# bitsauce/Carla-ppo

Measured on NVIDIA H100. Metric: VAE frames/sec @ batch 4096, higher is better.
Workload: dtype f32

## Files before the change

carla_ppo_b200/csrc/tc_wgrad.cu:

```cuda
#include "tc_common.cuh"
#include "wgrad.cuh"

namespace cpb {

namespace {

using namespace tc;

constexpr int CHUNK_KB = 4;

template <int BN, int PASSES>
struct TcWgCfg {
    static constexpr int B_TILE_BYTES = BN * TBK * 4;
    static constexpr int PARTS = PASSES == 3 ? 2 : 1;
    static constexpr int B_OFF = PARTS * A_TILE_BYTES;
    static constexpr int STAGE_BYTES = PARTS * A_TILE_BYTES + PARTS * B_TILE_BYTES;
    static constexpr int STAGES = (STAGE_BYTES * 4 <= 200 * 1024) ? 4 : 3;
    static constexpr int SMEM_BYTES = STAGES * STAGE_BYTES + 1024;
};

constexpr int kWgLoaderWarps = 8;
constexpr int kWgBWarps = 4;
constexpr int kWgThreads = (kWgLoaderWarps + kWgBWarps) * 32;

template <int BN, int PASSES>
__global__ void __maxnreg__(168)
tc_wgrad_kernel(const __grid_constant__ WgradParams p) {
    static_assert(PASSES == 3 || PASSES == 1, "3xTF32 or a single TF32 pass");
    using Cfg = TcWgCfg<BN, PASSES>;
    constexpr int STAGES = Cfg::STAGES;
    constexpr int B_TILE_BYTES = Cfg::B_TILE_BYTES;
    constexpr int B_OFF = Cfg::B_OFF;
    constexpr int STAGE_BYTES = Cfg::STAGE_BYTES;

    extern __shared__ uint8_t smem_raw[];
    __shared__ uint64_t full_bar[STAGES];
    __shared__ uint64_t empty_bar[STAGES];

    const int tid = threadIdx.x;
    const int warp = __shfl_sync(0xffffffffu, tid >> 5, 0), lane = tid & 31;
    const int i0 = blockIdx.x * TBM;
    const int j0 = blockIdx.y * BN;
    const int HoWo = p.Ho * p.Wo;
    const long long M = (long long)p.batch * HoWo;
    const long long m_begin = (long long)blockIdx.z * p.m_per_split;
    long long m_end = m_begin + p.m_per_split;
    if (m_end > M) m_end = M;
    const int nkb = m_end > m_begin ? 2 * (int)((m_end - m_begin + 2 * TBK - 1) / (2 * TBK)) : 0;

    const uint32_t smem_base = (smem_u32(smem_raw) + 1023u) & ~1023u;
    if (tid == 0) {
#pragma unroll
        for (int s = 0; s < STAGES; ++s) { mbar_init(&full_bar[s], kWgLoaderWarps + kWgBWarps); mbar_init(&empty_bar[s], kWgLoaderWarps); }
        asm volatile("fence.mbarrier_init.release.cluster;" ::: "memory");
    }
    __syncthreads();
    constexpr int BQ = BN / 4;
    const int len = (int)(m_end - m_begin);
    auto store_t = [&](uint32_t tile_hi, uint32_t tile_lo, const float4* x, const uint32_t* so) {
        const float xs[4][4] = {{x[0].x, x[1].x, x[2].x, x[3].x}, {x[0].y, x[1].y, x[2].y, x[3].y},
                                {x[0].z, x[1].z, x[2].z, x[3].z}, {x[0].w, x[1].w, x[2].w, x[3].w}};
#pragma unroll
        for (int c = 0; c < 4; ++c) {
            if constexpr (PASSES == 3) {
                float4 hi, lo;
                split_tf32(xs[c][0], hi.x, lo.x); split_tf32(xs[c][1], hi.y, lo.y);
                split_tf32(xs[c][2], hi.z, lo.z); split_tf32(xs[c][3], hi.w, lo.w);
                asm volatile("st.shared.v4.f32 [%0], {%1,%2,%3,%4};" ::"r"(tile_hi + so[c]), "f"(hi.x), "f"(hi.y), "f"(hi.z), "f"(hi.w) : "memory");
                asm volatile("st.shared.v4.f32 [%0], {%1,%2,%3,%4};" ::"r"(tile_lo + so[c]), "f"(lo.x), "f"(lo.y), "f"(lo.z), "f"(lo.w) : "memory");
            } else {
                asm volatile("st.shared.v4.b32 [%0], {%1,%2,%3,%4};" ::"r"(tile_hi + so[c]), "r"(round_tf32(xs[c][0])),
                             "r"(round_tf32(xs[c][1])), "r"(round_tf32(xs[c][2])), "r"(round_tf32(xs[c][3])) : "memory");
            }
        }
    };

    if (warp >= kWgLoaderWarps) {
        constexpr int NCGH = BQ >= 8 ? BQ / 8 : 1;
        const int r = (tid - kWgLoaderWarps * 32) >> 3;
        const int cgb = (r % NCGH) * 8 + (lane & 7);
        const int mb0 = r / NCGH;
        const bool active = mb0 < 8;
        uint32_t soffb[4];
#pragma unroll
        for (int c = 0; c < 4; ++c) {
            const int rb = BQ * c + cgb;
            soffb[c] = (uint32_t)((rb >> 3) * 1024 + (rb & 7) * 128 + ((mb0 ^ (rb & 7)) << 4));
        }
        int relB = mb0 * 4;
        const float* bptr = p.small + (m_begin + relB) * p.J + j0 + cgb * 4;
        auto load_b = [&](float4* xb) {
#pragma unroll
            for (int j = 0; j < 4; ++j) {
                xb[j] = make_float4(0.f, 0.f, 0.f, 0.f);
                if (active && relB + j < len) xb[j] = __ldg(reinterpret_cast<const float4*>(bptr + j * p.J));
            }
            relB += TBK;
            bptr += TBK * p.J;
        };
        float4 xb0[4], xb1[4];
        int sS = 0;
        uint32_t phS = 1;
        auto step_b = [&](int kb, float4* xb) {
            const uint32_t stage = smem_base + sS * STAGE_BYTES + B_OFF;
            mbar_wait(&empty_bar[sS], phS);
            if (active) store_t(stage, stage + B_TILE_BYTES, xb, soffb);
            fence_async_smem();
            __syncwarp();
            if (lane == 0) mbar_arrive(&full_bar[sS]);
            if (kb + 2 < nkb) load_b(xb);
            if (++sS == STAGES) { sS = 0; phS ^= 1u; }
        };
        if (nkb > 0) load_b(xb0);
        if (nkb > 1) load_b(xb1);
        for (int kb = 0; kb < nkb; kb += 2) {
            step_b(kb, xb0);
            step_b(kb + 1, xb1);
        }
    } else {
        const int cg = (warp & 3) * 8 + (lane & 7);
        const int mb = (warp >> 2) * 4 + (lane >> 3);
        const int a_i = i0 + cg * 4;
        const bool a_col_ok = a_i < p.I;
        long long a_coloff = 0;
        if (a_col_ok) {
            const int tap = a_i / p.run;
            a_coloff = p.tap_off[tap] + (a_i - tap * p.run);
        }
        uint32_t soff[4];
#pragma unroll
        for (int c = 0; c < 4; ++c) {
            const int ra = 32 * c + cg;
            soff[c] = (uint32_t)((ra >> 3) * 1024 + (ra & 7) * 128 + ((mb ^ (ra & 7)) << 4));
        }

        const uint32_t wo_magic = (uint32_t)((0x100000000ull + (uint32_t)p.Wo - 1) / (uint32_t)p.Wo);
        const int dx = p.sstride * p.big_pitch;
        const int drow = (p.sstride * p.Wb - p.Wo * p.sstride) * p.big_pitch;
        const int dimg = (int)(p.big_img - (long long)p.Ho * p.sstride * p.Wb * p.big_pitch);
        int nL, remL, relL = mb * 4;
        {
            const long long m = m_begin + relL;
            nL = (int)(m / HoWo);
            remL = (int)(m - (long long)nL * HoWo);
        }
        auto load_regs = [&](float4* areg) {
            int oy = (int)__umulhi((uint32_t)remL, wo_magic);
            int ox = remL - oy * p.Wo;
            uint32_t off = (uint32_t)nL * (uint32_t)p.big_img + (uint32_t)((oy * p.sstride * p.Wb + ox * p.sstride) * p.big_pitch) + (uint32_t)a_coloff;
#pragma unroll
            for (int j = 0; j < 4; ++j) {
                const bool v = relL + j < len;
                areg[j] = make_float4(0.f, 0.f, 0.f, 0.f);
                if (v && a_col_ok) areg[j] = __ldg(reinterpret_cast<const float4*>(p.big + off));
                off += (uint32_t)dx;
                if (++ox == p.Wo) { ox = 0; off += (uint32_t)drow; if (++oy == p.Ho) { oy = 0; off += (uint32_t)dimg; } }
            }
            relL += TBK;
            remL += TBK;
            while (remL >= HoWo) { remL -= HoWo; ++nL; }
        };

        constexpr int HALF = BN / 2;
        const int wg = warp >> 2;
        constexpr int DN = PASSES == 3 ? BN : HALF;
        float acc[HALF];
        float d[DN];
#pragma unroll
        for (int i = 0; i < HALF; ++i) acc[i] = 0.f;
#pragma unroll
        for (int i = 0; i < DN; ++i) d[i] = 0.f;

        float4 xa0[4], xa1[4];
        int sS = 0;
        uint32_t phS = 1;
        int prev = -1;
        auto step = [&](int kb, float4* xa) {
            const int s = sS;
            const uint32_t stage = smem_base + s * STAGE_BYTES;
            mbar_wait(&empty_bar[s], phS);
            store_t(stage, stage + A_TILE_BYTES, xa, soff);
            fence_async_smem();
            __syncwarp();
            if (lane == 0) mbar_arrive(&full_bar[s]);
            if (kb + 2 < nkb) load_regs(xa);
            mbar_wait(&full_bar[s], (uint32_t)((kb / STAGES) & 1));
            const uint64_t a_hi = make_desc(stage + wg * (A_TILE_BYTES / 2));
            const uint64_t a_lo = make_desc(stage + A_TILE_BYTES + wg * (A_TILE_BYTES / 2));
            const uint64_t b_hi = make_desc(stage + B_OFF);
            const uint64_t b_lo = make_desc(stage + B_OFF + B_TILE_BYTES);
            wgmma_fence();
#pragma unroll
            for (int ks = 0; ks < TBK / 8; ++ks) {
                const uint64_t adv = (uint64_t)(ks * 2);
                const uint32_t keep = ((kb % CHUNK_KB) | ks) != 0 ? 1u : 0u;
                wgmma_tf32<BN>(d, a_hi + adv, b_hi + adv, keep);
                if constexpr (PASSES == 3) {
                    wgmma_tf32<BN>(d + HALF, a_hi + adv, b_lo + adv, keep);
                    wgmma_tf32<BN>(d + HALF, a_lo + adv, b_hi + adv, 1u);
                }
            }
            wgmma_commit();
            if (kb % CHUNK_KB == CHUNK_KB - 1 || kb == nkb - 1) {
                wgmma_wait<0>();
                fence_regs<DN>(d);
                if (lane == 0) {
                    if (prev >= 0) mbar_arrive(&empty_bar[prev]);
                    mbar_arrive(&empty_bar[s]);
                }
                prev = -1;
#pragma unroll
                for (int i = 0; i < HALF; ++i) {
                    acc[i] += d[i];
                    if constexpr (PASSES == 3) acc[i] += d[HALF + i];
                }
            } else {
                if (prev >= 0) {
                    wgmma_wait<1>();
                    if (lane == 0) mbar_arrive(&empty_bar[prev]);
                }
                prev = s;
            }
            if (++sS == STAGES) { sS = 0; phS ^= 1u; }
        };
        if (nkb > 0) load_regs(xa0);
        if (nkb > 1) load_regs(xa1);
        for (int kb = 0; kb < nkb; kb += 2) {
            step(kb, xa0);
            step(kb + 1, xa1);
        }
        wgmma_wait<0>();

#pragma unroll
        for (int h = 0; h < 2; ++h) {
            const int rho = wg * 64 + (warp & 3) * 16 + (lane >> 2) + 8 * h;
            const int i = i0 + 4 * (rho & 31) + (rho >> 5);
            if (i >= p.I) continue;
            float* out = p.partial + ((long long)blockIdx.z * p.I + i) * p.J + j0;
#pragma unroll
            for (int j = 0; j < BN / 8; ++j)
#pragma unroll
                for (int c = 0; c < 2; ++c) {
                    const int rb = 8 * j + 2 * (lane & 3) + c;
                    out[4 * (rb % BQ) + rb / BQ] = acc[4 * j + 2 * h + c];
                }
        }
    }
}
template <int BN, int PASSES>
int32_t tc_wg_launch(const WgradParams& p, cudaStream_t stream) {
    dim3 grid((unsigned)cdiv(p.I, TBM), (unsigned)(p.J / BN), (unsigned)p.splits);
    tc_wgrad_kernel<BN, PASSES><<<grid, kWgThreads, TcWgCfg<BN, PASSES>::SMEM_BYTES, stream>>>(p);
    CPB_LAUNCHED();
    return CPB_OK;
}

template <int BN, int PASSES>
int32_t tc_wg_init_one() {
    CPB_CUDA(cudaFuncSetAttribute(tc_wgrad_kernel<BN, PASSES>, cudaFuncAttributeMaxDynamicSharedMemorySize, TcWgCfg<BN, PASSES>::SMEM_BYTES));
    return CPB_OK;
}

int tc_wg_bn(int J) { return J % 64 == 0 ? 64 : 32; }

}

int32_t tc_wgrad_init() {
    CPB_TRY((tc_wg_init_one<32, 3>()));
    CPB_TRY((tc_wg_init_one<64, 3>()));
    CPB_TRY((tc_wg_init_one<32, 1>()));
    CPB_TRY((tc_wg_init_one<64, 1>()));
    return CPB_OK;
}

bool tc_wgrad_supported(int I, int J, int run) { return run % 4 == 0 && J % 32 == 0 && I >= 128; }

int tc_wgrad_pick_splits(int I, int J, long long M) {
    const long long tiles = (long long)cdiv(I, TBM) * (J / tc_wg_bn(J));
    long long splits = kTcWaveCtas / tiles;
    const long long max_splits = (M + 1023) / 1024;
    if (splits > max_splits) splits = max_splits;
    if (splits < 1) splits = 1;
    return (int)splits;
}

int32_t launch_tc_wgrad(const WgradParams& p, cudaStream_t stream) {
    CPB_REQUIRE(tc_wgrad_supported(p.I, p.J, p.run) && p.I == p.ntaps * p.run, "tc_wgrad: unsupported problem (I=%d J=%d)", p.I, p.J);
    CPB_REQUIRE(p.m_per_split % TBK == 0 && p.splits >= 1, "tc_wgrad: bad split");
    CPB_REQUIRE((long long)p.batch * p.big_img < (1ll << 31) && p.m_per_split < (1ll << 30) && p.Wo < 65536 && p.Ho * p.Wo < 65536,
                "tc_wgrad: tensor too large for 32-bit offsets");
    CPB_REQUIRE(p.passes == 3 || p.passes == 1, "tc_wgrad: passes must be 3 or 1, got %d", p.passes);
    if (p.passes == 1) return tc_wg_bn(p.J) == 64 ? tc_wg_launch<64, 1>(p, stream) : tc_wg_launch<32, 1>(p, stream);
    return tc_wg_bn(p.J) == 64 ? tc_wg_launch<64, 3>(p, stream) : tc_wg_launch<32, 3>(p, stream);
}

}
```

Baseline: 54730.

## Load wgrad A tile via cp.async and feed wgmma from registers

The weight-gradient kernel now has four dedicated producer warps that bring the im2col A operand into shared memory with cp.async, signalled through the mbarrier, and also stage the B operand. Eight consumer warps read A from shared memory, split or round it to TF32 in registers, and issue register-sourced wgmma instead of descriptor-based A. The goal is to take the A global loads and TF32 conversion off the MMA warps' critical path and to halve A shared memory per stage, which allows up to 8 pipeline stages. In exchange, the consumer now waits on every wgmma group instead of keeping one in flight, adds register pressure for the A fragments, and redoes the TF32 split on every k-block.

```diff
diff --git a/carla_ppo_b200/csrc/tc_wgrad.cu b/carla_ppo_b200/csrc/tc_wgrad.cu
--- a/carla_ppo_b200/csrc/tc_wgrad.cu
+++ b/carla_ppo_b200/csrc/tc_wgrad.cu
@@ -13,15 +13,16 @@
 struct TcWgCfg {
     static constexpr int B_TILE_BYTES = BN * TBK * 4;
     static constexpr int PARTS = PASSES == 3 ? 2 : 1;
-    static constexpr int B_OFF = PARTS * A_TILE_BYTES;
-    static constexpr int STAGE_BYTES = PARTS * A_TILE_BYTES + PARTS * B_TILE_BYTES;
-    static constexpr int STAGES = (STAGE_BYTES * 4 <= 200 * 1024) ? 4 : 3;
+    static constexpr int B_OFF = A_TILE_BYTES;
+    static constexpr int STAGE_BYTES = A_TILE_BYTES + PARTS * B_TILE_BYTES;
+    static constexpr int STAGES = (192 * 1024) / STAGE_BYTES < 8 ? (192 * 1024) / STAGE_BYTES : 8;
     static constexpr int SMEM_BYTES = STAGES * STAGE_BYTES + 1024;
 };
 
-constexpr int kWgLoaderWarps = 8;
-constexpr int kWgBWarps = 4;
-constexpr int kWgThreads = (kWgLoaderWarps + kWgBWarps) * 32;
+constexpr int kWgMmaWarps = 8;
+constexpr int kWgLoaderWarps = 4;
+constexpr int kWgLoaderThreads = kWgLoaderWarps * 32;
+constexpr int kWgThreads = (kWgMmaWarps + kWgLoaderWarps) * 32;
 
 template <int BN, int PASSES>
 __global__ void __maxnreg__(168)
@@ -51,118 +52,120 @@
     const uint32_t smem_base = (smem_u32(smem_raw) + 1023u) & ~1023u;
     if (tid == 0) {
 #pragma unroll
-        for (int s = 0; s < STAGES; ++s) { mbar_init(&full_bar[s], kWgLoaderWarps + kWgBWarps); mbar_init(&empty_bar[s], kWgLoaderWarps); }
+        for (int s = 0; s < STAGES; ++s) { mbar_init(&full_bar[s], kWgLoaderThreads + kWgLoaderWarps); mbar_init(&empty_bar[s], kWgMmaWarps); }
         asm volatile("fence.mbarrier_init.release.cluster;" ::: "memory");
     }
     __syncthreads();
-    constexpr int BQ = BN / 4;
     const int len = (int)(m_end - m_begin);
-    auto store_t = [&](uint32_t tile_hi, uint32_t tile_lo, const float4* x, const uint32_t* so) {
-        const float xs[4][4] = {{x[0].x, x[1].x, x[2].x, x[3].x}, {x[0].y, x[1].y, x[2].y, x[3].y},
-                                {x[0].z, x[1].z, x[2].z, x[3].z}, {x[0].w, x[1].w, x[2].w, x[3].w}};
-#pragma unroll
-        for (int c = 0; c < 4; ++c) {
-            if constexpr (PASSES == 3) {
-                float4 hi, lo;
-                split_tf32(xs[c][0], hi.x, lo.x); split_tf32(xs[c][1], hi.y, lo.y);
-                split_tf32(xs[c][2], hi.z, lo.z); split_tf32(xs[c][3], hi.w, lo.w);
-                asm volatile("st.shared.v4.f32 [%0], {%1,%2,%3,%4};" ::"r"(tile_hi + so[c]), "f"(hi.x), "f"(hi.y), "f"(hi.z), "f"(hi.w) : "memory");
-                asm volatile("st.shared.v4.f32 [%0], {%1,%2,%3,%4};" ::"r"(tile_lo + so[c]), "f"(lo.x), "f"(lo.y), "f"(lo.z), "f"(lo.w) : "memory");
-            } else {
-                asm volatile("st.shared.v4.b32 [%0], {%1,%2,%3,%4};" ::"r"(tile_hi + so[c]), "r"(round_tf32(xs[c][0])),
-                             "r"(round_tf32(xs[c][1])), "r"(round_tf32(xs[c][2])), "r"(round_tf32(xs[c][3])) : "memory");
-            }
-        }
-    };
-
-    if (warp >= kWgLoaderWarps) {
-        constexpr int NCGH = BQ >= 8 ? BQ / 8 : 1;
-        const int r = (tid - kWgLoaderWarps * 32) >> 3;
-        const int cgb = (r % NCGH) * 8 + (lane & 7);
-        const int mb0 = r / NCGH;
-        const bool active = mb0 < 8;
-        uint32_t soffb[4];
-#pragma unroll
-        for (int c = 0; c < 4; ++c) {
-            const int rb = BQ * c + cgb;
-            soffb[c] = (uint32_t)((rb >> 3) * 1024 + (rb & 7) * 128 + ((mb0 ^ (rb & 7)) << 4));
-        }
-        int relB = mb0 * 4;
-        const float* bptr = p.small + (m_begin + relB) * p.J + j0 + cgb * 4;
-        auto load_b = [&](float4* xb) {
-#pragma unroll
-            for (int j = 0; j < 4; ++j) {
-                xb[j] = make_float4(0.f, 0.f, 0.f, 0.f);
-                if (active && relB + j < len) xb[j] = __ldg(reinterpret_cast<const float4*>(bptr + j * p.J));
-            }
-            relB += TBK;
-            bptr += TBK * p.J;
-        };
-        float4 xb0[4], xb1[4];
-        int sS = 0;
-        uint32_t phS = 1;
-        auto step_b = [&](int kb, float4* xb) {
-            const uint32_t stage = smem_base + sS * STAGE_BYTES + B_OFF;
-            mbar_wait(&empty_bar[sS], phS);
-            if (active) store_t(stage, stage + B_TILE_BYTES, xb, soffb);
-            fence_async_smem();
-            __syncwarp();
-            if (lane == 0) mbar_arrive(&full_bar[sS]);
-            if (kb + 2 < nkb) load_b(xb);
-            if (++sS == STAGES) { sS = 0; phS ^= 1u; }
-        };
-        if (nkb > 0) load_b(xb0);
-        if (nkb > 1) load_b(xb1);
-        for (int kb = 0; kb < nkb; kb += 2) {
-            step_b(kb, xb0);
-            step_b(kb + 1, xb1);
-        }
-    } else {
-        const int cg = (warp & 3) * 8 + (lane & 7);
-        const int mb = (warp >> 2) * 4 + (lane >> 3);
-        const int a_i = i0 + cg * 4;
+
+    if (warp >= kWgMmaWarps) {
+        const int tl = tid - kWgMmaWarps * 32;
+        const int pg = tl >> 5;
+        const int a_i = i0 + 4 * lane;
         const bool a_col_ok = a_i < p.I;
         long long a_coloff = 0;
         if (a_col_ok) {
             const int tap = a_i / p.run;
             a_coloff = p.tap_off[tap] + (a_i - tap * p.run);
         }
-        uint32_t soff[4];
-#pragma unroll
-        for (int c = 0; c < 4; ++c) {
-            const int ra = 32 * c + cg;
-            soff[c] = (uint32_t)((ra >> 3) * 1024 + (ra & 7) * 128 + ((mb ^ (ra & 7)) << 4));
-        }
-
+        const uint32_t a_dst0 = (uint32_t)(8 * pg * 512);
         const uint32_t wo_magic = (uint32_t)((0x100000000ull + (uint32_t)p.Wo - 1) / (uint32_t)p.Wo);
         const int dx = p.sstride * p.big_pitch;
         const int drow = (p.sstride * p.Wb - p.Wo * p.sstride) * p.big_pitch;
         const int dimg = (int)(p.big_img - (long long)p.Ho * p.sstride * p.Wb * p.big_pitch);
-        int nL, remL, relL = mb * 4;
+        int nA, remA, relA = 8 * pg;
         {
-            const long long m = m_begin + relL;
-            nL = (int)(m / HoWo);
-            remL = (int)(m - (long long)nL * HoWo);
-        }
-        auto load_regs = [&](float4* areg) {
-            int oy = (int)__umulhi((uint32_t)remL, wo_magic);
-            int ox = remL - oy * p.Wo;
-            uint32_t off = (uint32_t)nL * (uint32_t)p.big_img + (uint32_t)((oy * p.sstride * p.Wb + ox * p.sstride) * p.big_pitch) + (uint32_t)a_coloff;
-#pragma unroll
-            for (int j = 0; j < 4; ++j) {
-                const bool v = relL + j < len;
-                areg[j] = make_float4(0.f, 0.f, 0.f, 0.f);
-                if (v && a_col_ok) areg[j] = __ldg(reinterpret_cast<const float4*>(p.big + off));
+            const long long m = m_begin + relA;
+            nA = (int)(m / HoWo);
+            remA = (int)(m - (long long)nA * HoWo);
+        }
+        auto issue_a = [&](uint32_t stage, uint64_t* full) {
+            int oy = (int)__umulhi((uint32_t)remA, wo_magic);
+            int ox = remA - oy * p.Wo;
+            uint32_t off = (uint32_t)nA * (uint32_t)p.big_img + (uint32_t)((oy * p.sstride * p.Wb + ox * p.sstride) * p.big_pitch) + (uint32_t)a_coloff;
+#pragma unroll
+            for (int j = 0; j < 8; ++j) {
+                const bool v = relA + j < len && a_col_ok;
+                const uint32_t dst = stage + a_dst0 + j * 512 + ((lane ^ ((j & 1) << 2)) << 4);
+                asm volatile("cp.async.cg.shared.global [%0], [%1], 16, %2;" ::"r"(dst), "l"(p.big + (v ? off : 0u)), "r"(v ? 16u : 0u) : "memory");
                 off += (uint32_t)dx;
                 if (++ox == p.Wo) { ox = 0; off += (uint32_t)drow; if (++oy == p.Ho) { oy = 0; off += (uint32_t)dimg; } }
             }
-            relL += TBK;
-            remL += TBK;
-            while (remL >= HoWo) { remL -= HoWo; ++nL; }
-        };
-
+            asm volatile("cp.async.mbarrier.arrive.noinc.shared::cta.b64 [%0];" ::"r"(smem_u32(full)) : "memory");
+            relA += TBK;
+            remA += TBK;
+            while (remA >= HoWo) { remA -= HoWo; ++nA; }
+        };
+
+        constexpr int BQ = BN / 4;
+        constexpr int NCGH = BQ >= 8 ? BQ / 8 : 1;
+        const int r = tl >> 3;
+        const int cgb = (r % NCGH) * 8 + (lane & 7);
+        const int mb0 = r / NCGH;
+        const bool active = mb0 < 8;
+        uint32_t soffb[4];
+#pragma unroll
+        for (int c = 0; c < 4; ++c) {
+            const int rb = BQ * c + cgb;
+            soffb[c] = (uint32_t)((rb >> 3) * 1024 + (rb & 7) * 128 + ((mb0 ^ (rb & 7)) << 4));
+        }
+        auto store_t = [&](uint32_t tile_hi, uint32_t tile_lo, const float4* x) {
+            const float xs[4][4] = {{x[0].x, x[1].x, x[2].x, x[3].x}, {x[0].y, x[1].y, x[2].y, x[3].y},
+                                    {x[0].z, x[1].z, x[2].z, x[3].z}, {x[0].w, x[1].w, x[2].w, x[3].w}};
+#pragma unroll
+            for (int c = 0; c < 4; ++c) {
+                if constexpr (PASSES == 3) {
+                    float4 hi, lo;
+                    split_tf32(xs[c][0], hi.x, lo.x); split_tf32(xs[c][1], hi.y, lo.y);
+                    split_tf32(xs[c][2], hi.z, lo.z); split_tf32(xs[c][3], hi.w, lo.w);
+                    asm volatile("st.shared.v4.f32 [%0], {%1,%2,%3,%4};" ::"r"(tile_hi + soffb[c]), "f"(hi.x), "f"(hi.y), "f"(hi.z), "f"(hi.w) : "memory");
+                    asm volatile("st.shared.v4.f32 [%0], {%1,%2,%3,%4};" ::"r"(tile_lo + soffb[c]), "f"(lo.x), "f"(lo.y), "f"(lo.z), "f"(lo.w) : "memory");
+                } else {
+                    asm volatile("st.shared.v4.b32 [%0], {%1,%2,%3,%4};" ::"r"(tile_hi + soffb[c]), "r"(round_tf32(xs[c][0])),
+                                 "r"(round_tf32(xs[c][1])), "r"(round_tf32(xs[c][2])), "r"(round_tf32(xs[c][3])) : "memory");
+                }
+            }
+        };
+        int relB = mb0 * 4;
+        const float* bptr = p.small + (m_begin + relB) * p.J + j0 + cgb * 4;
+        auto load_b = [&](float4* xb) {
+#pragma unroll
+            for (int j = 0; j < 4; ++j) {
+                xb[j] = make_float4(0.f, 0.f, 0.f, 0.f);
+                if (active && relB + j < len) xb[j] = __ldg(reinterpret_cast<const float4*>(bptr + j * p.J));
+            }
+            relB += TBK;
+            bptr += TBK * p.J;
+        };
+        float4 xb0[4], xb1[4], xb2[4], xb3[4];
+        int sS = 0;
+        uint32_t phS = 1;
+        auto step = [&](int kb, float4* xb) {
+            if (kb >= nkb) return;
+            const uint32_t stage = smem_base + sS * STAGE_BYTES;
+            mbar_wait(&empty_bar[sS], phS);
+            issue_a(stage, &full_bar[sS]);
+            if (active) store_t(stage + B_OFF, stage + B_OFF + B_TILE_BYTES, xb);
+            fence_async_smem();
+            __syncwarp();
+            if (lane == 0) mbar_arrive(&full_bar[sS]);
+            if (kb + 4 < nkb) load_b(xb);
+            if (++sS == STAGES) { sS = 0; phS ^= 1u; }
+        };
+        if (nkb > 0) load_b(xb0);
+        if (nkb > 1) load_b(xb1);
+        if (nkb > 2) load_b(xb2);
+        if (nkb > 3) load_b(xb3);
+        for (int kb = 0; kb < nkb; kb += 4) {
+            step(kb, xb0);
+            step(kb + 1, xb1);
+            step(kb + 2, xb2);
+            step(kb + 3, xb3);
+        }
+    } else {
+        const int g = lane >> 2, t = lane & 3;
+        const uint32_t a_rd = (uint32_t)(t * 512 + (((4 * warp + (g >> 1)) ^ ((t & 1) << 2)) << 4) + (g & 1) * 8);
         constexpr int HALF = BN / 2;
-        const int wg = warp >> 2;
         constexpr int DN = PASSES == 3 ? BN : HALF;
         float acc[HALF];
         float d[DN];
@@ -171,22 +174,38 @@
 #pragma unroll
         for (int i = 0; i < DN; ++i) d[i] = 0.f;
 
-        float4 xa0[4], xa1[4];
-        int sS = 0;
-        uint32_t phS = 1;
-        int prev = -1;
-        auto step = [&](int kb, float4* xa) {
-            const int s = sS;
+        int s = 0;
+        uint32_t ph = 0;
+        for (int kb = 0; kb < nkb; ++kb) {
+            mbar_wait(&full_bar[s], ph);
             const uint32_t stage = smem_base + s * STAGE_BYTES;
-            mbar_wait(&empty_bar[s], phS);
-            store_t(stage, stage + A_TILE_BYTES, xa, soff);
-            fence_async_smem();
-            __syncwarp();
-            if (lane == 0) mbar_arrive(&full_bar[s]);
-            if (kb + 2 < nkb) load_regs(xa);
-            mbar_wait(&full_bar[s], (uint32_t)((kb / STAGES) & 1));
-            const uint64_t a_hi = make_desc(stage + wg * (A_TILE_BYTES / 2));
-            const uint64_t a_lo = make_desc(stage + A_TILE_BYTES + wg * (A_TILE_BYTES / 2));
+            uint32_t ah[TBK / 8][4], al[TBK / 8][4];
+#pragma unroll
+            for (int ks = 0; ks < TBK / 8; ++ks)
+#pragma unroll
+                for (int h = 0; h < 2; ++h) {
+                    float2 x;
+                    asm volatile("ld.shared.v2.f32 {%0,%1}, [%2];" : "=f"(x.x), "=f"(x.y) : "r"(stage + a_rd + (4 * h + 8 * ks) * 512));
+#pragma unroll
+                    for (int v = 0; v < 2; ++v) {
+                        const float xv = v ? x.y : x.x;
+                        if constexpr (PASSES == 3) {
+                            float hi, lo;
+                            split_tf32(xv, hi, lo);
+                            ah[ks][2 * h + v] = __float_as_uint(hi);
+                            al[ks][2 * h + v] = __float_as_uint(lo);
+                        } else {
+                            ah[ks][2 * h + v] = round_tf32(xv);
+                        }
+                    }
+                }
+#pragma unroll
+            for (int ks = 0; ks < TBK / 8; ++ks)
+#pragma unroll
+                for (int i = 0; i < 4; ++i) {
+                    if constexpr (PASSES == 3) asm volatile("" : "+r"(ah[ks][i]), "+r"(al[ks][i]));
+                    else asm volatile("" : "+r"(ah[ks][i]));
+                }
             const uint64_t b_hi = make_desc(stage + B_OFF);
             const uint64_t b_lo = make_desc(stage + B_OFF + B_TILE_BYTES);
             wgmma_fence();
@@ -194,54 +213,37 @@
             for (int ks = 0; ks < TBK / 8; ++ks) {
                 const uint64_t adv = (uint64_t)(ks * 2);
                 const uint32_t keep = ((kb % CHUNK_KB) | ks) != 0 ? 1u : 0u;
-                wgmma_tf32<BN>(d, a_hi + adv, b_hi + adv, keep);
+                wgmma_tf32_rs<BN>(d, ah[ks], b_hi + adv, keep);
                 if constexpr (PASSES == 3) {
-                    wgmma_tf32<BN>(d + HALF, a_hi + adv, b_lo + adv, keep);
-                    wgmma_tf32<BN>(d + HALF, a_lo + adv, b_hi + adv, 1u);
+                    wgmma_tf32_rs<BN>(d + HALF, ah[ks], b_lo + adv, keep);
+                    wgmma_tf32_rs<BN>(d + HALF, al[ks], b_hi + adv, 1u);
                 }
             }
             wgmma_commit();
+            wgmma_wait<0>();
+            fence_regs<DN>(d);
+            if (lane == 0) mbar_arrive(&empty_bar[s]);
             if (kb % CHUNK_KB == CHUNK_KB - 1 || kb == nkb - 1) {
-                wgmma_wait<0>();
-                fence_regs<DN>(d);
-                if (lane == 0) {
-                    if (prev >= 0) mbar_arrive(&empty_bar[prev]);
-                    mbar_arrive(&empty_bar[s]);
-                }
-                prev = -1;
 #pragma unroll
                 for (int i = 0; i < HALF; ++i) {
                     acc[i] += d[i];
                     if constexpr (PASSES == 3) acc[i] += d[HALF + i];
                 }
-            } else {
-                if (prev >= 0) {
-                    wgmma_wait<1>();
-                    if (lane == 0) mbar_arrive(&empty_bar[prev]);
-                }
-                prev = s;
-            }
-            if (++sS == STAGES) { sS = 0; phS ^= 1u; }
-        };
-        if (nkb > 0) load_regs(xa0);
-        if (nkb > 1) load_regs(xa1);
-        for (int kb = 0; kb < nkb; kb += 2) {
-            step(kb, xa0);
-            step(kb + 1, xa1);
-        }
-        wgmma_wait<0>();
-
+            }
+            if (++s == STAGES) { s = 0; ph ^= 1u; }
+        }
+
+        constexpr int BQ = BN / 4;
 #pragma unroll
         for (int h = 0; h < 2; ++h) {
-            const int rho = wg * 64 + (warp & 3) * 16 + (lane >> 2) + 8 * h;
-            const int i = i0 + 4 * (rho & 31) + (rho >> 5);
+            const int i = i0 + 16 * warp + 2 * g + h;
             if (i >= p.I) continue;
             float* out = p.partial + ((long long)blockIdx.z * p.I + i) * p.J + j0;
 #pragma unroll
             for (int j = 0; j < BN / 8; ++j)
 #pragma unroll
                 for (int c = 0; c < 2; ++c) {
-                    const int rb = 8 * j + 2 * (lane & 3) + c;
+                    const int rb = 8 * j + 2 * t + c;
                     out[4 * (rb % BQ) + rb / BQ] = acc[4 * j + 2 * h + c];
                 }
         }
```

Result: faster. 58920 (median of 6 runs) (+7.7%).
